# FocoosAI/focoos

Hardware: NVIDIA H100
Metric: images/sec fai-detr-l bs=32 640x640 inference (higher is better)
Workload: dtype f32 (storage and accumulation; every conv/linear product = 3 f16 wgmma products, error ~2^-21)

## Files before the change

### focoos_b200/csrc/conv_tc.cu

```cuda
#include <cuda.h>

#include <cstdlib>
#include <type_traits>

#include "common.cuh"
#include "tma.cuh"
#include "wgmma.cuh"

namespace fb200 {

namespace tc {

constexpr int BLOCK_M = 128;
constexpr int STAGING_BYTES = BLOCK_M * 128;
constexpr int NUM_THREADS = 384;
constexpr int CONSUMER_WARPS = 8;

struct PairOut { __half hi, lo; };
template <typename T> struct is_pair { static constexpr bool value = false; };
template <> struct is_pair<PairOut> { static constexpr bool value = true; };

struct KParams {
  const float* scale; const float* bias; const void* res;
  int act, Cout;
  int KH, KW, pad, cchunks;
  int w_batched;
  int lo_off;
  int w_seg;
  int BW, BH, tiles_w, tiles_h;
  int Ho, Wo;
  int x_pitch;
  int stride2;
  int num_k_blocks;
  int n_tiles, total_tiles;
  float* rowmax;
};

__device__ __forceinline__ void consumer_bar() { asm volatile("bar.sync 1, 256;" ::: "memory"); }

template <int BLOCK_K>
__device__ __forceinline__ uint64_t make_smem_desc(uint32_t smem_addr) {
  uint64_t d = 0;
  d |= (uint64_t)((smem_addr & 0x3FFFFu) >> 4);
  d |= (uint64_t)1 << 16;
  d |= (uint64_t)((8 * BLOCK_K * 2) >> 4) << 32;
  d |= (uint64_t)(BLOCK_K == 64 ? 1 : 2) << 62;
  return d;
}

template <bool GELU>
__device__ __forceinline__ float act1(float v, int act) {
  if constexpr (GELU) return 0.5f * v * (1.f + erff(v * 0.70710678118654752440f));
  switch (act & 15) {
    case FB200_ACT_RELU: return fmaxf(v, 0.f);
    case FB200_ACT_SILU: return __fdividef(v, 1.f + __expf(-v));
    default: return v;
  }
}

__device__ __forceinline__ void atomic_max_float(float* addr, float v) {
  if (v >= 0.f) atomicMax(reinterpret_cast<int*>(addr), __float_as_int(v));
  else atomicMin(reinterpret_cast<unsigned int*>(addr), __float_as_uint(v));
}

struct AccThread {
  int ct;
  int g;
  int r0;
  int cq;
};
__device__ __forceinline__ AccThread acc_thread() {
  const int ct = threadIdx.x - 128, lane = threadIdx.x & 31;
  return {ct, ct >> 7, (ct >> 7) * 64 + ((ct & 127) >> 5) * 16 + (lane >> 2), 2 * (lane & 3)};
}

template <typename TOut>
__device__ __forceinline__ int staging_offset(int row, int lc) {
  if constexpr (is_pair<TOut>::value) return row * 64 + ((((lc >> 3) ^ ((row >> 1) & 3)) << 4) | ((lc & 7) * 2));
  else if constexpr (sizeof(TOut) == 2) return row * 128 + ((((lc >> 3) ^ (row & 7)) << 4) | ((lc & 7) * 2));
  else return row * 128 + ((((lc >> 2) ^ (row & 7)) << 4) | ((lc & 3) * 4));
}

template <typename TOut>
__device__ __forceinline__ void staging_store(uint8_t* stg, int off, float v0, float v1) {
  if constexpr (is_pair<TOut>::value) {
    const __half2 hi = __floats2half2_rn(v0, v1);
    const float2 hf = __half22float2(hi);
    *reinterpret_cast<__half2*>(stg + off) = hi;
    *reinterpret_cast<__half2*>(stg + STAGING_BYTES / 2 + off) = __floats2half2_rn(v0 - hf.x, v1 - hf.y);
  } else if constexpr (sizeof(TOut) == 2) {
    *reinterpret_cast<__half2*>(stg + off) = __floats2half2_rn(v0, v1);
  } else {
    *reinterpret_cast<float2*>(stg + off) = make_float2(v0, v1);
  }
}

template <int NSTG, typename F>
__device__ __forceinline__ void staging_open(int ct, F&& then) {
  if (ct == 0) {
    tma_store_wait_read<NSTG - 1>();
    then();
  }
  consumer_bar();
}
template <typename TOut>
__device__ __forceinline__ void staging_close(int ct, const uint8_t* stg, const CUtensorMap* tmap_d, const CUtensorMap* tmap_d2, int n, int w0, int h0, int img) {
  fence_proxy_async();
  consumer_bar();
  if (ct == 0) {
    tma_store_4d(tmap_d, stg, n, w0, h0, img);
    if constexpr (is_pair<TOut>::value) tma_store_4d(tmap_d2, stg + STAGING_BYTES / 2, n, w0, h0, img);
    tma_store_commit();
  }
}

template <int BLOCK_K, bool FS> __host__ __device__ constexpr int a_stage_bytes() { return (FS ? 2 : 1) * BLOCK_M * BLOCK_K * 2; }
template <int BLOCK_N, int BLOCK_K, bool FS> __host__ __device__ constexpr int b_stage_bytes() { return (FS ? 2 : 1) * BLOCK_N * BLOCK_K * 2; }
template <int BLOCK_N, int STAGES, int BLOCK_K, int NSTG, bool FS> constexpr int smem_bytes() {
  return STAGES * (a_stage_bytes<BLOCK_K, FS>() + b_stage_bytes<BLOCK_N, BLOCK_K, FS>()) + NSTG * STAGING_BYTES + (2 * STAGES + 1) * 8 + 1024 ;
}

template <int BLOCK_N, int STAGES, typename TOut, int BLOCK_K, int NSTG, bool GELU, bool FS>
__global__ void __launch_bounds__(NUM_THREADS, 1)
conv_tc_kernel(const __grid_constant__ CUtensorMap tmap_a, const __grid_constant__ CUtensorMap tmap_b,
               const __grid_constant__ CUtensorMap tmap_d, const __grid_constant__ CUtensorMap tmap_r,
               const __grid_constant__ CUtensorMap tmap_d2, const __grid_constant__ CUtensorMap tmap_r2, const KParams p) {
  constexpr bool PAIR = is_pair<TOut>::value;
  static_assert(BLOCK_K == 32 || BLOCK_K == 64, "one swizzle row per channel chunk");
  extern __shared__ __align__(1024) uint8_t smem_raw[];
  uint8_t* smem = reinterpret_cast<uint8_t*>((reinterpret_cast<uintptr_t>(smem_raw) + 1023) & ~uintptr_t(1023));
  constexpr int A_STAGE_BYTES = a_stage_bytes<BLOCK_K, FS>();
  constexpr int B_STAGE_BYTES = b_stage_bytes<BLOCK_N, BLOCK_K, FS>();
  constexpr int A_HALF = BLOCK_M * BLOCK_K * 2;
  constexpr int B_HALF = BLOCK_N * BLOCK_K * 2;
  uint8_t* smem_a = smem;
  uint8_t* smem_b = smem + STAGES * A_STAGE_BYTES;
  uint8_t* staging = smem_b + STAGES * B_STAGE_BYTES;
  uint64_t* full_bar = reinterpret_cast<uint64_t*>(staging + NSTG * STAGING_BYTES);
  uint64_t* empty_bar = full_bar + STAGES;
  uint64_t* res_bar = empty_bar + STAGES;

  constexpr int CHUNK_COLS = 128 / (int)sizeof(TOut);
  constexpr int NCHUNKS = (BLOCK_N + CHUNK_COLS - 1) / CHUNK_COLS;
  constexpr int RES_SLOTS_A = A_STAGE_BYTES / STAGING_BYTES;
  constexpr int RES_SLOTS = RES_SLOTS_A + B_STAGE_BYTES / STAGING_BYTES;
  constexpr bool RES_RING = RES_SLOTS > 0;
  const bool res_ring = RES_RING && p.res != nullptr && p.rowmax == nullptr;
  auto res_slot = [&](int s, int slot) -> uint8_t* {
    return slot < RES_SLOTS_A ? smem_a + s * A_STAGE_BYTES + slot * STAGING_BYTES : smem_b + s * B_STAGE_BYTES + (slot - RES_SLOTS_A) * STAGING_BYTES;
  };
  auto chunks_of = [&](int n0) { return min(NCHUNKS, (p.Cout - n0 + CHUNK_COLS - 1) / CHUNK_COLS); };

  const int warp = threadIdx.x >> 5, lane = threadIdx.x & 31;
  if (threadIdx.x == 0) {
    asm volatile("prefetch.tensormap [%0];" ::"l"(&tmap_a) : "memory");
    asm volatile("prefetch.tensormap [%0];" ::"l"(&tmap_b) : "memory");
    asm volatile("prefetch.tensormap [%0];" ::"l"(&tmap_d) : "memory");
    for (int i = 0; i < STAGES; ++i) { mbar_init(&full_bar[i], 1); mbar_init(&empty_bar[i], CONSUMER_WARPS); }
    if constexpr (!RES_RING) mbar_init(res_bar, 1);
    fence_barrier_init();
  }
  __syncthreads();
  const int tiles_per_img = p.tiles_w * p.tiles_h;
  struct TileXY { int n0, img, h0, w0; };
  auto tile_of = [&](int t) {
    TileXY r;
    r.n0 = (t % p.n_tiles) * BLOCK_N;
    const int mt = t / p.n_tiles;
    r.img = mt / tiles_per_img;
    const int rem = mt - r.img * tiles_per_img;
    r.h0 = (rem / p.tiles_w) * p.BH;
    r.w0 = (rem % p.tiles_w) * p.BW;
    return r;
  };

  if (warp < 4) {
    if (threadIdx.x != 0) return;
    const uint32_t a_bytes = (uint32_t)(p.BW * p.BH * BLOCK_K * 2);
    auto load_a = [&](uint64_t* bar, void* dst, int c, int kh, int kw, int h0, int w0, int img) {
      if (!p.stride2) {
        tma_load_4d(&tmap_a, bar, dst, c, w0 + kw - p.pad, h0 + kh - p.pad, img);
      } else if (p.stride2 == 2) {
        tma_load_4d(&tmap_a, bar, dst, c, 2 * w0 + kw - p.pad, 2 * h0 + kh - p.pad, img);
      } else {
        const int th = kh - p.pad, tw = kw - p.pad;
        tma_load_5d(&tmap_a, bar, dst, (tw & 1) * p.x_pitch + c, w0 + (tw >> 1), th & 1, h0 + (th >> 1), img);
      }
    };
    auto load_b = [&](uint64_t* bar, void* dst, int k, int n0, int img) {
      if (p.w_batched) tma_load_3d(&tmap_b, bar, dst, k, n0, img);
      else tma_load_2d(&tmap_b, bar, dst, k, n0);
    };
    int stage = 0;
    uint32_t phase = 0;
    for (int t = blockIdx.x; t < p.total_tiles; t += gridDim.x) {
      const TileXY tc = tile_of(t);
      for (int kb = 0; kb < p.num_k_blocks; ++kb) {
        mbar_wait(&empty_bar[stage], phase ^ 1);
        const int tap = kb / p.cchunks, cc = kb - tap * p.cchunks;
        const int kh = tap / p.KW, kw = tap - kh * p.KW;
        uint8_t* dst_a = smem_a + stage * A_STAGE_BYTES;
        uint8_t* dst_b = smem_b + stage * B_STAGE_BYTES;
        if constexpr (FS) {
          const int k_hi = tap * 3 * p.w_seg + cc * BLOCK_K, k_lo = k_hi + p.w_seg;
          mbar_arrive_expect_tx(&full_bar[stage], 2u * a_bytes + (uint32_t)B_STAGE_BYTES);
          load_a(&full_bar[stage], dst_a, cc * BLOCK_K, kh, kw, tc.h0, tc.w0, tc.img);
          load_a(&full_bar[stage], dst_a + A_HALF, p.lo_off + cc * BLOCK_K, kh, kw, tc.h0, tc.w0, tc.img);
          load_b(&full_bar[stage], dst_b, k_hi, tc.n0, tc.img);
          load_b(&full_bar[stage], dst_b + B_HALF, k_lo, tc.n0, tc.img);
        } else {
          mbar_arrive_expect_tx(&full_bar[stage], a_bytes + (uint32_t)B_STAGE_BYTES);
          load_a(&full_bar[stage], dst_a, cc * BLOCK_K, kh, kw, tc.h0, tc.w0, tc.img);
          load_b(&full_bar[stage], dst_b, kb * BLOCK_K, tc.n0, tc.img);
        }
        if (++stage == STAGES) { stage = 0; phase ^= 1; }
      }
      if constexpr (RES_RING) if (res_ring) {
        const int nch = chunks_of(tc.n0);
        for (int ch = 0; ch < nch; ++ch) {
          const int slot = ch % RES_SLOTS;
          if (slot == 0) {
            mbar_wait(&empty_bar[stage], phase ^ 1);
            mbar_arrive_expect_tx(&full_bar[stage], (uint32_t)(min(RES_SLOTS, nch - ch) * p.BW * p.BH * 128));
          }
          uint8_t* dst = res_slot(stage, slot);
          tma_load_4d(&tmap_r, &full_bar[stage], dst, tc.n0 + ch * CHUNK_COLS, tc.w0, tc.h0, tc.img);
          if constexpr (PAIR) tma_load_4d(&tmap_r2, &full_bar[stage], dst + STAGING_BYTES / 2, tc.n0 + ch * CHUNK_COLS, tc.w0, tc.h0, tc.img);
          if (slot == RES_SLOTS - 1 || ch == nch - 1) {
            if (++stage == STAGES) { stage = 0; phase ^= 1; }
          }
        }
      }
    }
    return;
  }

  const AccThread th = acc_thread();
  constexpr int NACC = BLOCK_N / 2;
  const bool post = (p.act & FB200_ACT_RESIDUAL_AFTER) != 0;
  const bool has_res = p.res != nullptr;
  float acc[NACC];
  int stage = 0;
  uint32_t phase = 0, res_phase = 0, chunk_ctr = 0;
  for (int t = blockIdx.x; t < p.total_tiles; t += gridDim.x) {
    const TileXY tc = tile_of(t);
    int prev = -1;
    for (int kb = 0; kb < p.num_k_blocks; ++kb) {
      mbar_wait(&full_bar[stage], phase);
      const uint32_t sa = smem_u32(smem_a + stage * A_STAGE_BYTES) + (uint32_t)(th.g * 64 * BLOCK_K * 2);
      const uint32_t sb = smem_u32(smem_b + stage * B_STAGE_BYTES);
      const uint64_t da = make_smem_desc<BLOCK_K>(sa), db = make_smem_desc<BLOCK_K>(sb);
      wgmma_fence();
#pragma unroll
      for (int k = 0; k < BLOCK_K / 16; ++k) {
        const uint64_t ko = (uint64_t)(k * 2);
        Wgmma<BLOCK_N, 0>::mma(acc, da + ko, db + ko, (kb > 0 || k > 0) ? 1u : 0u);
        if constexpr (FS) {
          const uint64_t da_lo = make_smem_desc<BLOCK_K>(sa + A_HALF), db_lo = make_smem_desc<BLOCK_K>(sb + B_HALF);
          Wgmma<BLOCK_N, 0>::mma(acc, da + ko, db_lo + ko, 1u);
          Wgmma<BLOCK_N, 0>::mma(acc, da_lo + ko, db + ko, 1u);
        }
      }
      wgmma_commit();
      wgmma_wait<1>();
      if (prev >= 0 && lane == 0) mbar_arrive(&empty_bar[prev]);
      prev = stage;
      if (++stage == STAGES) { stage = 0; phase ^= 1; }
    }
    wgmma_wait<0>();
    if (prev >= 0 && lane == 0) mbar_arrive(&empty_bar[prev]);

    auto scale_of = [&](int n) { return (p.scale && n < p.Cout) ? __ldg(p.scale + n) : 1.f; };
    auto bias_of = [&](int n) { return (p.bias && n < p.Cout) ? __ldg(p.bias + n) : 0.f; };
    auto row_valid = [&](int row, int64_t& pix) {
      const int bh = row / p.BW, bw = row - bh * p.BW;
      const int ho = tc.h0 + bh, wo = tc.w0 + bw;
      pix = ((int64_t)tc.img * p.Ho + ho) * p.Wo + wo;
      return row < p.BW * p.BH && ho < p.Ho && wo < p.Wo;
    };
    if (p.rowmax) {
      float m[2] = {-INFINITY, -INFINITY};
#pragma unroll
      for (int j = 0; j < BLOCK_N / 8; ++j) {
#pragma unroll
        for (int e = 0; e < 2; ++e) {
          const int n = tc.n0 + 8 * j + th.cq + e;
          if (n < p.Cout) {
            const float s = scale_of(n), b = bias_of(n);
            m[0] = fmaxf(m[0], fmaf(acc[4 * j + e], s, b));
            m[1] = fmaxf(m[1], fmaf(acc[4 * j + 2 + e], s, b));
          }
        }
      }
#pragma unroll
      for (int h = 0; h < 2; ++h) {
        m[h] = fmaxf(m[h], __shfl_xor_sync(0xffffffffu, m[h], 1));
        m[h] = fmaxf(m[h], __shfl_xor_sync(0xffffffffu, m[h], 2));
        int64_t pix;
        if ((lane & 3) == 0 && row_valid(th.r0 + 8 * h, pix)) atomic_max_float(p.rowmax + pix, m[h]);
      }
      continue;
    }
    const int nch = chunks_of(tc.n0);
#pragma unroll
    for (int ch = 0; ch < NCHUNKS; ++ch) {
      const int c0 = ch * CHUNK_COLS;
      if (ch >= nch) break;
      uint8_t* stg = staging + (chunk_ctr % NSTG) * STAGING_BYTES;
      const uint8_t* res = stg;
      staging_open<NSTG>(th.ct, [&] {
        if constexpr (!RES_RING) if (has_res) {
          mbar_arrive_expect_tx(res_bar, (uint32_t)(p.BW * p.BH * 128));
          tma_load_4d(&tmap_r, res_bar, stg, tc.n0 + c0, tc.w0, tc.h0, tc.img);
          if constexpr (PAIR) tma_load_4d(&tmap_r2, res_bar, stg + STAGING_BYTES / 2, tc.n0 + c0, tc.w0, tc.h0, tc.img);
        }
      });
      if constexpr (RES_RING) {
        if (res_ring) {
          if (ch % RES_SLOTS == 0) mbar_wait(&full_bar[stage], phase);
          res = res_slot(stage, ch % RES_SLOTS);
        }
      } else if (has_res) {
        mbar_wait(res_bar, res_phase);
        res_phase ^= 1;
      }
#pragma unroll
      for (int jj = 0; jj < CHUNK_COLS / 8; ++jj) {
        const int j = c0 / 8 + jj;
        if (j >= BLOCK_N / 8) break;
        const int lc = 8 * jj + th.cq;
        const int n = tc.n0 + c0 + lc;
        const float s0 = scale_of(n), s1 = scale_of(n + 1), b0 = bias_of(n), b1 = bias_of(n + 1);
#pragma unroll
        for (int h = 0; h < 2; ++h) {
          const int row = th.r0 + 8 * h;
          float v0 = fmaf(acc[4 * j + 2 * h], s0, b0), v1 = fmaf(acc[4 * j + 2 * h + 1], s1, b1);
          const int off = staging_offset<TOut>(row, lc);
          auto add_residual = [&]() {
            if (!has_res) return;
            if constexpr (PAIR) {
              const float2 fh = __half22float2(*reinterpret_cast<const __half2*>(res + off));
              const float2 fl = __half22float2(*reinterpret_cast<const __half2*>(res + STAGING_BYTES / 2 + off));
              v0 += fh.x + fl.x;
              v1 += fh.y + fl.y;
            } else if constexpr (sizeof(TOut) == 2) {
              const float2 f = __half22float2(*reinterpret_cast<const __half2*>(res + off));
              v0 += f.x;
              v1 += f.y;
            } else {
              const float2 f = *reinterpret_cast<const float2*>(res + off);
              v0 += f.x;
              v1 += f.y;
            }
          };
          if (!post) add_residual();
          v0 = act1<GELU>(v0, p.act);
          v1 = act1<GELU>(v1, p.act);
          if (post) add_residual();
          staging_store<TOut>(stg, off, v0, v1);
        }
      }
      if constexpr (RES_RING) {
        if (res_ring && (ch % RES_SLOTS == RES_SLOTS - 1 || ch == nch - 1)) {
          __syncwarp();
          if (lane == 0) mbar_arrive(&empty_bar[stage]);
          if (++stage == STAGES) { stage = 0; phase ^= 1; }
        }
      }
      staging_close<TOut>(th.ct, stg, &tmap_d, &tmap_d2, tc.n0 + c0, tc.w0, tc.h0, tc.img);
      ++chunk_ctr;
    }
  }
  if (th.ct == 0) tma_store_wait_all();
}

constexpr int SC_BW = 16, SC_BH = 8;
constexpr int SC_BOX_ROWS = SC_BW * (SC_BH + 2);
constexpr int SC_BOX_BYTES = SC_BOX_ROWS * 64;
constexpr int SC_STAGE_BYTES = 2 * 3 * SC_BOX_BYTES;
constexpr int SC_STAGES = 2;
template <int BLOCK_N> __host__ __device__ constexpr int sc_w_bytes() { return 9 * 2 * BLOCK_N * 64; }
template <int BLOCK_N> constexpr int sc_smem_bytes() {
  return sc_w_bytes<BLOCK_N>() + SC_STAGES * SC_STAGE_BYTES + 2 * STAGING_BYTES + (2 * SC_STAGES + 1) * 8 + 1024 ;
}

template <int BLOCK_N, typename TOut>
__global__ void __launch_bounds__(NUM_THREADS, 1)
conv_tc_smallc_kernel(const __grid_constant__ CUtensorMap tmap_a, const __grid_constant__ CUtensorMap tmap_b,
                      const __grid_constant__ CUtensorMap tmap_d, const __grid_constant__ CUtensorMap tmap_d2, const KParams p) {
  constexpr int W_BYTES = sc_w_bytes<BLOCK_N>();
  constexpr int W_TAP = 2 * BLOCK_N * 64;
  extern __shared__ __align__(1024) uint8_t smem_raw[];
  uint8_t* smem = reinterpret_cast<uint8_t*>((reinterpret_cast<uintptr_t>(smem_raw) + 1023) & ~uintptr_t(1023));
  uint8_t* smem_w = smem;
  uint8_t* smem_a = smem_w + W_BYTES;
  uint8_t* staging = smem_a + SC_STAGES * SC_STAGE_BYTES;
  uint64_t* full_bar = reinterpret_cast<uint64_t*>(staging + 2 * STAGING_BYTES);
  uint64_t* empty_bar = full_bar + SC_STAGES;
  uint64_t* w_bar = empty_bar + SC_STAGES;
  constexpr int CHUNK_COLS = 32;
  constexpr int NCHUNKS = BLOCK_N / CHUNK_COLS;

  const int warp = threadIdx.x >> 5, lane = threadIdx.x & 31;
  if (threadIdx.x == 0) {
    asm volatile("prefetch.tensormap [%0];" ::"l"(&tmap_a) : "memory");
    asm volatile("prefetch.tensormap [%0];" ::"l"(&tmap_d) : "memory");
    for (int i = 0; i < SC_STAGES; ++i) { mbar_init(&full_bar[i], 1); mbar_init(&empty_bar[i], CONSUMER_WARPS); }
    mbar_init(w_bar, 1);
    fence_barrier_init();
  }
  __syncthreads();
  const int tiles_per_img = p.tiles_w * p.tiles_h;
  struct TileXY { int img, h0, w0; };
  auto tile_of = [&](int t) {
    TileXY r;
    r.img = t / tiles_per_img;
    const int rem = t - r.img * tiles_per_img;
    r.h0 = (rem / p.tiles_w) * SC_BH;
    r.w0 = (rem % p.tiles_w) * SC_BW;
    return r;
  };

  if (warp < 4) {
    if (threadIdx.x != 0) return;
    mbar_arrive_expect_tx(w_bar, (uint32_t)W_BYTES);
    for (int tap = 0; tap < 9; ++tap) {
      tma_load_2d(&tmap_b, w_bar, smem_w + tap * W_TAP, tap * 3 * p.w_seg, 0);
      tma_load_2d(&tmap_b, w_bar, smem_w + tap * W_TAP + W_TAP / 2, tap * 3 * p.w_seg + p.w_seg, 0);
    }
    int stage = 0;
    uint32_t phase = 0;
    for (int t = blockIdx.x; t < p.total_tiles; t += gridDim.x) {
      const TileXY tc = tile_of(t);
      mbar_wait(&empty_bar[stage], phase ^ 1);
      mbar_arrive_expect_tx(&full_bar[stage], (uint32_t)SC_STAGE_BYTES);
      uint8_t* dst = smem_a + stage * SC_STAGE_BYTES;
      for (int kw = 0; kw < 3; ++kw) {
        tma_load_4d(&tmap_a, &full_bar[stage], dst + kw * SC_BOX_BYTES, 0, tc.w0 + kw - 1, tc.h0 - 1, tc.img);
        tma_load_4d(&tmap_a, &full_bar[stage], dst + (3 + kw) * SC_BOX_BYTES, p.lo_off, tc.w0 + kw - 1, tc.h0 - 1, tc.img);
      }
      if (++stage == SC_STAGES) { stage = 0; phase ^= 1; }
    }
    return;
  }

  const AccThread th = acc_thread();
  float acc[BLOCK_N / 2];
  float sc[BLOCK_N / 4], bi[BLOCK_N / 4];
#pragma unroll
  for (int j = 0; j < BLOCK_N / 8; ++j)
#pragma unroll
    for (int e = 0; e < 2; ++e) {
      const int n = 8 * j + th.cq + e;
      sc[2 * j + e] = p.scale ? __ldg(p.scale + n) : 1.f;
      bi[2 * j + e] = p.bias ? __ldg(p.bias + n) : 0.f;
    }
  mbar_wait(w_bar, 0);
  const uint32_t sw = smem_u32(smem_w);
  int stage = 0;
  uint32_t phase = 0, chunk_ctr = 0;
  for (int t = blockIdx.x; t < p.total_tiles; t += gridDim.x) {
    const TileXY tc = tile_of(t);
    mbar_wait(&full_bar[stage], phase);
    const uint32_t sa = smem_u32(smem_a + stage * SC_STAGE_BYTES) + (uint32_t)(th.g * 64 * 64);
    wgmma_fence();
#pragma unroll
    for (int tap = 0; tap < 9; ++tap) {
      const int kh = tap / 3, kw = tap - 3 * (tap / 3);
      const uint32_t a_tap = sa + (uint32_t)(kw * SC_BOX_BYTES + kh * SC_BW * 64);
      const uint64_t da = make_smem_desc<32>(a_tap), da_lo = make_smem_desc<32>(a_tap + 3 * SC_BOX_BYTES);
      const uint64_t db = make_smem_desc<32>(sw + tap * W_TAP), db_lo = make_smem_desc<32>(sw + tap * W_TAP + W_TAP / 2);
#pragma unroll
      for (int k = 0; k < 2; ++k) {
        const uint64_t ko = (uint64_t)(k * 2);
        Wgmma<BLOCK_N, 0>::mma(acc, da + ko, db + ko, (tap > 0 || k > 0) ? 1u : 0u);
        Wgmma<BLOCK_N, 0>::mma(acc, da + ko, db_lo + ko, 1u);
        Wgmma<BLOCK_N, 0>::mma(acc, da_lo + ko, db + ko, 1u);
      }
    }
    wgmma_commit();
    wgmma_wait<0>();
    if (lane == 0) mbar_arrive(&empty_bar[stage]);
    if (++stage == SC_STAGES) { stage = 0; phase ^= 1; }

#pragma unroll
    for (int ch = 0; ch < NCHUNKS; ++ch) {
      uint8_t* stg = staging + (chunk_ctr & 1) * STAGING_BYTES;
      staging_open<2>(th.ct, [] {});
#pragma unroll
      for (int jj = 0; jj < CHUNK_COLS / 8; ++jj) {
        const int j = ch * (CHUNK_COLS / 8) + jj;
        const int lc = 8 * jj + th.cq;
#pragma unroll
        for (int h = 0; h < 2; ++h) {
          const int row = th.r0 + 8 * h;
          const float v0 = act1<false>(fmaf(acc[4 * j + 2 * h], sc[2 * j], bi[2 * j]), p.act);
          const float v1 = act1<false>(fmaf(acc[4 * j + 2 * h + 1], sc[2 * j + 1], bi[2 * j + 1]), p.act);
          staging_store<TOut>(stg, staging_offset<TOut>(row, lc), v0, v1);
        }
      }
      staging_close<TOut>(th.ct, stg, &tmap_d, &tmap_d2, ch * CHUNK_COLS, tc.w0, tc.h0, tc.img);
      ++chunk_ctr;
    }
  }
  if (th.ct == 0) tma_store_wait_all();
}

static void choose_tile(int Ho, int Wo, int* BW, int* BH) {
  double best = -1.0;
  for (int bw = 1; bw <= (Wo < 128 ? Wo : 128); ++bw) {
    int bh = 128 / bw;
    if (bh > Ho) bh = Ho;
    if (bh < 1) continue;
    const double tiles = (double)((Wo + bw - 1) / bw) * (double)((Ho + bh - 1) / bh);
    const double eff = (double)Wo * Ho / (tiles * 128.0);
    if (eff > best + 1e-9 || (eff > best - 1e-9 && bw > *BW)) { best = eff; *BW = bw; *BH = bh; }
  }
}

struct OutMaps { CUtensorMap d, d2, r, r2; };
static int encode_out_maps(OutMaps* m, const ConvParams& p, int Wo, int Ho, int B, int BW, int BH, uint64_t batch_stride) {
  const bool pair = p.out_dtype == FB200_F16PAIR, f32 = p.out_dtype == FB200_F32;
  const CUtensorMapDataType dt = f32 ? CU_TENSOR_MAP_DATA_TYPE_FLOAT32 : CU_TENSOR_MAP_DATA_TYPE_FLOAT16;
  const int elt = f32 ? 4 : 2;
  const CUtensorMapSwizzle swz = pair ? CU_TENSOR_MAP_SWIZZLE_64B : CU_TENSOR_MAP_SWIZZLE_128B;
  const uint64_t OP = (uint64_t)p.out_pitch, RP = (uint64_t)p.res_pitch;
  const uint64_t dims[4] = {(uint64_t)p.Cout, (uint64_t)Wo, (uint64_t)Ho, (uint64_t)B};
  const uint64_t str[4] = {1, OP, OP * Wo, batch_stride}, rstr[4] = {1, RP, RP * Wo, RP * Wo * Ho};
  const uint32_t box[4] = {(uint32_t)(pair || f32 ? 32 : 64), (uint32_t)BW, (uint32_t)BH, 1};
  int rc = encode(&m->d, dt, elt, 4, p.out, dims, str, box, pair ? "conv_tc: D(hi)" : "conv_tc: D", swz);
  if (rc) return rc;
  m->d2 = m->d;
  if (pair) rc = encode(&m->d2, dt, elt, 4, static_cast<__half*>(p.out) + p.out_lo_off, dims, str, box, "conv_tc: D(lo)", swz);
  if (rc) return rc;
  m->r = m->d; m->r2 = m->d2;
  if (!p.res) return FB200_OK;
  rc = encode(&m->r, dt, elt, 4, const_cast<void*>(p.res), dims, rstr, box, pair ? "conv_tc: R(hi)" : "conv_tc: R", swz);
  if (rc || !pair) return rc;
  return encode(&m->r2, dt, elt, 4, const_cast<__half*>(static_cast<const __half*>(p.res)) + p.res_lo_off, dims, rstr, box, "conv_tc: R(lo)", swz);
}

static bool smallc_fits(const ConvParams& p) {
  return p.split3 && p.Cin == 3 * 32 && (p.Cout == 32 || p.Cout == 64) && p.KH == 3 && p.KW == 3 && p.stride == 1 && p.pad == 1 &&
         !p.res && !p.rowmax && p.w_bs == 0 && (p.out_dtype == FB200_F32 || p.out_dtype == FB200_F16PAIR);
}

static int conv2d_tc_smallc(const ConvParams& p, cudaStream_t st) {
  KParams kp{};
  kp.scale = p.scale; kp.bias = p.bias; kp.act = p.act; kp.Cout = p.Cout;
  kp.lo_off = (int)p.x_lo_off;
  kp.w_seg = 32;
  kp.tiles_w = (p.Wo + SC_BW - 1) / SC_BW; kp.tiles_h = (p.Ho + SC_BH - 1) / SC_BH; kp.Ho = p.Ho; kp.Wo = p.Wo;
  const int64_t total = (int64_t)p.B * kp.tiles_w * kp.tiles_h;
  if (total > 0x7fffffffLL) { set_error("conv_tc: too many tiles (%lld)", (long long)total); return FB200_ERR_UNSUPPORTED; }
  kp.total_tiles = (int)total;
  CUtensorMap ta, tb;
  OutMaps om;
  const uint64_t P = (uint64_t)p.x_pitch;
  {
    const uint64_t dims[4] = {(uint64_t)kp.lo_off + 32, (uint64_t)p.W, (uint64_t)p.H, (uint64_t)p.B};
    const uint64_t str[4] = {1, P, P * p.W, P * p.W * p.H};
    const uint32_t box[4] = {32, SC_BW, SC_BH + 2, 1};
    int rc = encode(&ta, CU_TENSOR_MAP_DATA_TYPE_FLOAT16, 2, 4, const_cast<void*>(p.x), dims, str, box, "conv_tc: A(patch)", CU_TENSOR_MAP_SWIZZLE_64B);
    if (rc) return rc;
  }
  {
    const uint64_t dims[2] = {(uint64_t)p.K, (uint64_t)p.Cout};
    const uint64_t str[2] = {1, (uint64_t)p.K};
    const uint32_t box[2] = {32, (uint32_t)p.Cout};
    int rc = encode(&tb, CU_TENSOR_MAP_DATA_TYPE_FLOAT16, 2, 2, const_cast<void*>(p.w), dims, str, box, "conv_tc: W", CU_TENSOR_MAP_SWIZZLE_64B);
    if (rc) return rc;
  }
  if (int rc = encode_out_maps(&om, p, p.Wo, p.Ho, p.B, SC_BW, SC_BH, (uint64_t)p.out_bs)) return rc;
  auto run = [&](auto blockn_tag, auto out_tag) -> int {
    constexpr int BN_ = decltype(blockn_tag)::value;
    return launch_persistent<conv_tc_smallc_kernel<BN_, decltype(out_tag)>, sc_smem_bytes<BN_>()>("conv_tc_smallc_kernel", kp.total_tiles, NUM_THREADS, st, ta, tb,
                                                                                                 om.d, om.d2, kp);
  };
  typedef std::integral_constant<int, 32> N32;
  typedef std::integral_constant<int, 64> N64;
  const bool outp = p.out_dtype == FB200_F16PAIR;
  if (p.Cout == 32) return outp ? run(N32{}, PairOut{}) : run(N32{}, float{});
  return outp ? run(N64{}, PairOut{}) : run(N64{}, float{});
}

}

bool conv2d_tc_supported(const ConvParams& p, int x_dtype, int out_dtype) {
  if (x_dtype != FB200_F16) return false;
  if (out_dtype != FB200_F16 && out_dtype != FB200_F32 && out_dtype != FB200_F16PAIR) return false;
  if (p.split3 && out_dtype == FB200_F16) return false;
  const int Clog = p.split3 ? p.Cin / 3 : p.Cin;
  if (out_dtype == FB200_F16PAIR) {
    if (!p.split3 || p.rowmax || p.w_bs != 0 || p.Cout % 8 != 0) return false;
    if ((p.out_lo_off * 2) % 16 != 0 || (p.out_pitch * 2) % 16 != 0 || (p.out_bs * 2) % 16 != 0) return false;
    if (p.res && ((p.res_lo_off * 2) % 16 != 0 || (p.res_pitch * 2) % 16 != 0 || p.Cout % 32 != 0)) return false;
  }
  if (p.split3 && (p.x_lo_off * 2) % 16 != 0) return false;
  if (Clog % 32 != 0 || p.x_pitch % 8 != 0) return false;
  if (p.split3 && p.Cin % 3 != 0) return false;
  if ((reinterpret_cast<uintptr_t>(p.x) | reinterpret_cast<uintptr_t>(p.w) | reinterpret_cast<uintptr_t>(p.out)) & 15) return false;
  const int oelt = out_dtype == FB200_F32 ? 4 : 2;
  if ((p.out_pitch * oelt) % 16 != 0) return false;
  if (!p.rowmax && (p.Cout * oelt) % 16 != 0) return false;
  if (p.res && ((p.res_pitch * oelt) % 16 != 0 || (reinterpret_cast<uintptr_t>(p.res) & 15))) return false;
  if (p.res && out_dtype != FB200_F16PAIR && p.Cout % (128 / oelt) != 0) return false;
  if (p.KH != p.KW) return false;
  if (p.w_bs != 0 && (p.w_bs * 2) % 16 != 0) return false;
  if ((p.act & 15) == FB200_ACT_GELU && (out_dtype != FB200_F16 || Clog % 64 != 0)) return false;
  if ((p.act & 15) == FB200_ACT_SIGMOID) return false;
  if ((p.out_bs * oelt) % 16 != 0) return false;
  if (p.stride == 1) return (2 * p.pad == p.KH - 1) || (p.KH == 1 && p.pad == 0);
  if (p.stride == 2) {
    if (p.KH == 3 && p.pad == 1) return true;
    return p.KH == 2 && p.pad == 0 && p.H % 2 == 0 && p.W % 2 == 0;
  }
  return false;
}

int conv2d_tc(const ConvParams& p, cudaStream_t st) {
  using namespace tc;
  if (smallc_fits(p)) return conv2d_tc_smallc(p, st);
  KParams kp;
  kp.scale = p.scale; kp.bias = p.bias; kp.res = p.res; kp.act = p.act; kp.Cout = p.Cout;
  kp.KH = p.KH; kp.KW = p.KW; kp.pad = p.pad;
  const int Clog = p.split3 ? p.Cin / 3 : p.Cin;
  const int BK = (Clog % 64 == 0) ? 64 : 32;
  kp.lo_off = p.split3 ? (int)p.x_lo_off : Clog;
  kp.w_seg = Clog;
  const CUtensorMapSwizzle swz = BK == 64 ? CU_TENSOR_MAP_SWIZZLE_128B : CU_TENSOR_MAP_SWIZZLE_64B;
  kp.cchunks = Clog / BK; kp.x_pitch = p.x_pitch;
  kp.stride2 = (p.stride != 2) ? 0 : (p.H % 2 == 0 && p.W % 2 == 0) ? 1 : 2;
  kp.num_k_blocks = p.KH * p.KW * kp.cchunks;
  int B = p.B, H = p.H, W = p.W, Ho = p.Ho, Wo = p.Wo;
  const bool flat = (p.KH == 1 && p.stride == 1 && p.out_bs == (int64_t)p.Ho * p.Wo * p.out_pitch) && p.w_bs == 0;
  kp.w_batched = p.w_bs != 0 ? 1 : 0;
  kp.rowmax = p.rowmax;
  if (flat) {
    if (p.M > 0x7fffffffLL) { set_error("conv_tc: M too large"); return FB200_ERR_UNSUPPORTED; }
    W = Wo = (int)p.M; H = Ho = 1; B = 1;
  }
  int BW = 1, BH = 1;
  choose_tile(Ho, Wo, &BW, &BH);
  kp.BW = BW; kp.BH = BH; kp.tiles_w = (Wo + BW - 1) / BW; kp.tiles_h = (Ho + BH - 1) / BH; kp.Ho = Ho; kp.Wo = Wo;
  const int64_t m_tiles = (int64_t)B * kp.tiles_w * kp.tiles_h;

  CUtensorMap ta, tb;
  OutMaps om;
  int rc;
  const uint64_t P = (uint64_t)p.x_pitch;
  if (!kp.stride2) {
    const uint64_t dims[4] = {(uint64_t)(p.split3 ? kp.lo_off + Clog : p.Cin), (uint64_t)W, (uint64_t)H, (uint64_t)B};
    const uint64_t str[4] = {1, P, P * W, P * W * H};
    const uint32_t box[4] = {(uint32_t)BK, (uint32_t)BW, (uint32_t)BH, 1};
    rc = encode(&ta, CU_TENSOR_MAP_DATA_TYPE_FLOAT16, 2, 4, const_cast<void*>(p.x), dims, str, box, "conv_tc: A", swz);
  } else if (kp.stride2 == 2) {
    const uint64_t dims[4] = {(uint64_t)(p.split3 ? kp.lo_off + Clog : p.Cin), (uint64_t)W, (uint64_t)H, (uint64_t)B};
    const uint64_t str[4] = {1, P, P * W, P * W * H};
    const uint32_t box[4] = {(uint32_t)BK, 2 * (uint32_t)BW, 2 * (uint32_t)BH, 1};
    const uint32_t estr[4] = {1, 2, 2, 1};
    rc = encode(&ta, CU_TENSOR_MAP_DATA_TYPE_FLOAT16, 2, 4, const_cast<void*>(p.x), dims, str, box, "conv_tc: A(s2 odd)", swz, estr);
  } else {
    const uint64_t dims[5] = {2 * P, (uint64_t)W / 2, 2, (uint64_t)H / 2, (uint64_t)B};
    const uint64_t str[5] = {1, 2 * P, P * W, 2 * P * W, P * W * H};
    const uint32_t box[5] = {(uint32_t)BK, (uint32_t)BW, 1, (uint32_t)BH, 1};
    rc = encode(&ta, CU_TENSOR_MAP_DATA_TYPE_FLOAT16, 2, 5, const_cast<void*>(p.x), dims, str, box, "conv_tc: A(s2)", swz);
  }
  if (rc) return rc;
  rc = encode_out_maps(&om, p, Wo, Ho, B, BW, BH, flat ? (uint64_t)p.out_pitch * Wo * Ho : (uint64_t)p.out_bs);
  if (rc) return rc;

  auto run = [&](auto blockn_tag, auto stages_tag, auto bk_tag, auto gelu_tag, auto fs_tag) -> int {
    constexpr bool FS_ = decltype(fs_tag)::value;
    constexpr int BN_ = decltype(blockn_tag)::value;
    constexpr int ST_ = decltype(stages_tag)::value;
    constexpr int BK_ = decltype(bk_tag)::value;
    constexpr int NS_ = 2;
    {
      const uint64_t dims[3] = {(uint64_t)p.K, (uint64_t)p.Cout, (uint64_t)p.B};
      const uint64_t str[3] = {1, (uint64_t)p.K, (uint64_t)p.w_bs};
      const uint32_t box[3] = {(uint32_t)BK_, (uint32_t)BN_, 1};
      int r2 = encode(&tb, CU_TENSOR_MAP_DATA_TYPE_FLOAT16, 2, p.w_bs ? 3 : 2, const_cast<void*>(p.w), dims, str, box, "conv_tc: W", swz);
      if (r2) return r2;
    }
    kp.n_tiles = (p.Cout + BN_ - 1) / BN_;
    const int64_t total = m_tiles * kp.n_tiles;
    if (total > 0x7fffffffLL) { set_error("conv_tc: too many tiles (%lld)", (long long)total); return FB200_ERR_UNSUPPORTED; }
    kp.total_tiles = (int)total;
    auto launch = [&](auto out_tag) -> int {
      return launch_persistent<conv_tc_kernel<BN_, ST_, decltype(out_tag), BK_, NS_, decltype(gelu_tag)::value, FS_>, smem_bytes<BN_, ST_, BK_, NS_, FS_>()>(
          "conv_tc_kernel", kp.total_tiles, NUM_THREADS, st, ta, tb, om.d, om.r, om.d2, om.r2, kp);
    };
    const bool outp = p.out_dtype == FB200_F16PAIR;
    if constexpr (decltype(gelu_tag)::value) return launch(__half{});
    else if constexpr (FS_) return outp ? launch(PairOut{}) : launch(float{});
    else {
      if (outp) { set_error("conv_tc: pair output is only produced by the fused-split configurations"); return FB200_ERR_UNSUPPORTED; }
      return p.out_dtype == FB200_F16 ? launch(__half{}) : launch(float{});
    }
  };
  using std::integral_constant;
  typedef std::false_type NF;
  typedef std::true_type FS;
  typedef integral_constant<int, 64> K64;
  typedef integral_constant<int, 32> K32;
  typedef integral_constant<int, 128> N128;
  typedef integral_constant<int, 64> N64;
  typedef integral_constant<int, 4> S4;
  typedef integral_constant<int, 3> S3;
  if ((p.act & 15) == FB200_ACT_GELU)
    return run(N128{}, S4{}, K64{}, std::true_type{}, NF{});
  if (p.split3) {
    if (BK == 64) {
      if (p.Cout > 64) return run(N128{}, S3{}, K64{}, std::false_type{}, FS{});
      return run(N64{}, S4{}, K64{}, std::false_type{}, FS{});
    }
    if (p.Cout > 64) return run(N128{}, S4{}, K32{}, std::false_type{}, FS{});
    return run(N64{}, S4{}, K32{}, std::false_type{}, FS{});
  }
  if (BK == 32) {
    if (p.Cout > 64) return run(N128{}, S4{}, K32{}, std::false_type{}, NF{});
    return run(N64{}, S4{}, K32{}, std::false_type{}, NF{});
  }
  if (p.Cout > 64) return run(N128{}, S4{}, K64{}, std::false_type{}, NF{});
  return run(N64{}, S4{}, K64{}, std::false_type{}, NF{});
}

}
```

Before: 905.1.

## Ping-pong consumer warpgroups with register reallocation in conv TC kernel

Measured after the change: 982.8, median of 6. 8.6% higher.

```diff
diff --git a/focoos_b200/csrc/conv_tc.cu b/focoos_b200/csrc/conv_tc.cu
--- a/focoos_b200/csrc/conv_tc.cu
+++ b/focoos_b200/csrc/conv_tc.cu
@@ -15,6 +15,8 @@
 constexpr int STAGING_BYTES = BLOCK_M * 128;
 constexpr int NUM_THREADS = 384;
 constexpr int CONSUMER_WARPS = 8;
+constexpr int GROUP_WARPS = 4;
+constexpr int PRODUCER_REGS = 40, CONSUMER_REGS = 232;
 
 struct PairOut { __half hi, lo; };
 template <typename T> struct is_pair { static constexpr bool value = false; };
@@ -36,7 +38,29 @@
   float* rowmax;
 };
 
-__device__ __forceinline__ void consumer_bar() { asm volatile("bar.sync 1, 256;" ::: "memory"); }
+__device__ __forceinline__ void bar_sync(int id, int n) { asm volatile("bar.sync %0, %1;" ::"r"(id), "r"(n) : "memory"); }
+__device__ __forceinline__ void bar_arrive(int id, int n) { asm volatile("bar.arrive %0, %1;" ::"r"(id), "r"(n) : "memory"); }
+template <int REGS> __device__ __forceinline__ void regs_dec() { asm volatile("setmaxnreg.dec.sync.aligned.u32 %0;" ::"n"(REGS)); }
+template <int REGS> __device__ __forceinline__ void regs_inc() { asm volatile("setmaxnreg.inc.sync.aligned.u32 %0;" ::"n"(REGS)); }
+
+__device__ __forceinline__ uint32_t sreg_tid() {
+  uint32_t v;
+  asm volatile("mov.u32 %0, %%tid.x;" : "=r"(v));
+  return v;
+}
+__device__ __forceinline__ int grid_ctas() {
+  uint32_t v;
+  asm volatile("mov.u32 %0, %%nctaid.x;" : "=r"(v));
+  return (int)v;
+}
+__device__ __forceinline__ int pp_row() { const uint32_t t = sreg_tid(); return (int)((t & 127) >> 5) * 16 + (int)((t & 31) >> 2); }
+__device__ __forceinline__ int pp_col() { return 2 * (int)(sreg_tid() & 3); }
+
+struct Team {
+  bool issuer;
+  int bar, n;
+  __device__ __forceinline__ void sync() const { bar_sync(bar, n); }
+};
 
 template <int BLOCK_K>
 __device__ __forceinline__ uint64_t make_smem_desc(uint32_t smem_addr) {
@@ -81,33 +105,36 @@
   else return row * 128 + ((((lc >> 2) ^ (row & 7)) << 4) | ((lc & 3) * 4));
 }
 
+__device__ __forceinline__ uint32_t h2_bits(__half2 h) { return *reinterpret_cast<uint32_t*>(&h); }
+__device__ __forceinline__ void sts_b32(uint32_t a, uint32_t v) { asm volatile("st.shared.b32 [%0], %1;" ::"r"(a), "r"(v) : "memory"); }
+__device__ __forceinline__ void sts_f2(uint32_t a, float x, float y) { asm volatile("st.shared.v2.f32 [%0], {%1, %2};" ::"r"(a), "f"(x), "f"(y) : "memory"); }
 template <typename TOut>
-__device__ __forceinline__ void staging_store(uint8_t* stg, int off, float v0, float v1) {
+__device__ __forceinline__ void staging_store(uint32_t stg, int off, float v0, float v1) {
   if constexpr (is_pair<TOut>::value) {
     const __half2 hi = __floats2half2_rn(v0, v1);
     const float2 hf = __half22float2(hi);
-    *reinterpret_cast<__half2*>(stg + off) = hi;
-    *reinterpret_cast<__half2*>(stg + STAGING_BYTES / 2 + off) = __floats2half2_rn(v0 - hf.x, v1 - hf.y);
+    sts_b32(stg + off, h2_bits(hi));
+    sts_b32(stg + STAGING_BYTES / 2 + off, h2_bits(__floats2half2_rn(v0 - hf.x, v1 - hf.y)));
   } else if constexpr (sizeof(TOut) == 2) {
-    *reinterpret_cast<__half2*>(stg + off) = __floats2half2_rn(v0, v1);
+    sts_b32(stg + off, h2_bits(__floats2half2_rn(v0, v1)));
   } else {
-    *reinterpret_cast<float2*>(stg + off) = make_float2(v0, v1);
+    sts_f2(stg + off, v0, v1);
   }
 }
 
 template <int NSTG, typename F>
-__device__ __forceinline__ void staging_open(int ct, F&& then) {
-  if (ct == 0) {
+__device__ __forceinline__ void staging_open(const Team& tm, F&& then) {
+  if (tm.issuer) {
     tma_store_wait_read<NSTG - 1>();
     then();
   }
-  consumer_bar();
+  tm.sync();
 }
 template <typename TOut>
-__device__ __forceinline__ void staging_close(int ct, const uint8_t* stg, const CUtensorMap* tmap_d, const CUtensorMap* tmap_d2, int n, int w0, int h0, int img) {
+__device__ __forceinline__ void staging_close(const Team& tm, const uint8_t* stg, const CUtensorMap* tmap_d, const CUtensorMap* tmap_d2, int n, int w0, int h0, int img) {
   fence_proxy_async();
-  consumer_bar();
-  if (ct == 0) {
+  tm.sync();
+  if (tm.issuer) {
     tma_store_4d(tmap_d, stg, n, w0, h0, img);
     if constexpr (is_pair<TOut>::value) tma_store_4d(tmap_d2, stg + STAGING_BYTES / 2, n, w0, h0, img);
     tma_store_commit();
@@ -127,6 +154,7 @@
                const __grid_constant__ CUtensorMap tmap_d2, const __grid_constant__ CUtensorMap tmap_r2, const KParams p) {
   constexpr bool PAIR = is_pair<TOut>::value;
   static_assert(BLOCK_K == 32 || BLOCK_K == 64, "one swizzle row per channel chunk");
+  static_assert(NSTG == 2, "one staging buffer per consumer warp-group");
   extern __shared__ __align__(1024) uint8_t smem_raw[];
   uint8_t* smem = reinterpret_cast<uint8_t*>((reinterpret_cast<uintptr_t>(smem_raw) + 1023) & ~uintptr_t(1023));
   constexpr int A_STAGE_BYTES = a_stage_bytes<BLOCK_K, FS>();
@@ -138,17 +166,9 @@
   uint8_t* staging = smem_b + STAGES * B_STAGE_BYTES;
   uint64_t* full_bar = reinterpret_cast<uint64_t*>(staging + NSTG * STAGING_BYTES);
   uint64_t* empty_bar = full_bar + STAGES;
-  uint64_t* res_bar = empty_bar + STAGES;
-
   constexpr int CHUNK_COLS = 128 / (int)sizeof(TOut);
   constexpr int NCHUNKS = (BLOCK_N + CHUNK_COLS - 1) / CHUNK_COLS;
-  constexpr int RES_SLOTS_A = A_STAGE_BYTES / STAGING_BYTES;
-  constexpr int RES_SLOTS = RES_SLOTS_A + B_STAGE_BYTES / STAGING_BYTES;
-  constexpr bool RES_RING = RES_SLOTS > 0;
-  const bool res_ring = RES_RING && p.res != nullptr && p.rowmax == nullptr;
-  auto res_slot = [&](int s, int slot) -> uint8_t* {
-    return slot < RES_SLOTS_A ? smem_a + s * A_STAGE_BYTES + slot * STAGING_BYTES : smem_b + s * B_STAGE_BYTES + (slot - RES_SLOTS_A) * STAGING_BYTES;
-  };
+  constexpr int ROW_BYTES = PAIR ? 64 : 128;
   auto chunks_of = [&](int n0) { return min(NCHUNKS, (p.Cout - n0 + CHUNK_COLS - 1) / CHUNK_COLS); };
 
   const int warp = threadIdx.x >> 5, lane = threadIdx.x & 31;
@@ -156,8 +176,7 @@
     asm volatile("prefetch.tensormap [%0];" ::"l"(&tmap_a) : "memory");
     asm volatile("prefetch.tensormap [%0];" ::"l"(&tmap_b) : "memory");
     asm volatile("prefetch.tensormap [%0];" ::"l"(&tmap_d) : "memory");
-    for (int i = 0; i < STAGES; ++i) { mbar_init(&full_bar[i], 1); mbar_init(&empty_bar[i], CONSUMER_WARPS); }
-    if constexpr (!RES_RING) mbar_init(res_bar, 1);
+    for (int i = 0; i < STAGES; ++i) { mbar_init(&full_bar[i], 1); mbar_init(&empty_bar[i], GROUP_WARPS); }
     fence_barrier_init();
   }
   __syncthreads();
@@ -175,6 +194,7 @@
   };
 
   if (warp < 4) {
+    regs_dec<PRODUCER_REGS>();
     if (threadIdx.x != 0) return;
     const uint32_t a_bytes = (uint32_t)(p.BW * p.BH * BLOCK_K * 2);
     auto load_a = [&](uint64_t* bar, void* dst, int c, int kh, int kw, int h0, int w0, int img) {
@@ -215,6 +235,250 @@
         }
         if (++stage == STAGES) { stage = 0; phase ^= 1; }
       }
+    }
+    return;
+  }
+
+  regs_inc<CONSUMER_REGS>();
+  const int g = (threadIdx.x - 128) >> 7;
+  const Team team{(threadIdx.x & 127) == 0, 2 + g, 128};
+  uint8_t* stg = staging + g * STAGING_BYTES;
+  constexpr int NACC = BLOCK_N / 2;
+  float acc[2][NACC];
+  int stage = 0;
+  uint32_t phase = 0;
+  for (int t = blockIdx.x + g * grid_ctas(); t < p.total_tiles; t += 2 * grid_ctas()) {
+    if (t != blockIdx.x) {
+      stage += p.num_k_blocks;
+      phase ^= (uint32_t)((stage / STAGES) & 1);
+      stage %= STAGES;
+      bar_sync(4 + g, 256);
+    }
+    for (int kb = 0; kb < p.num_k_blocks; ++kb) {
+      mbar_wait(&full_bar[stage], phase);
+      const uint32_t sa = smem_u32(smem_a + stage * A_STAGE_BYTES);
+      const uint32_t sb = smem_u32(smem_b + stage * B_STAGE_BYTES);
+      const uint64_t da = make_smem_desc<BLOCK_K>(sa), db = make_smem_desc<BLOCK_K>(sb);
+      wgmma_fence();
+#pragma unroll
+      for (int k = 0; k < BLOCK_K / 16; ++k) {
+        const uint64_t ko = (uint64_t)(k * 2);
+#pragma unroll
+        for (int hf = 0; hf < 2; ++hf) {
+          const uint64_t dah = da + (uint64_t)(hf * 64 * BLOCK_K * 2 / 16) + ko;
+          Wgmma<BLOCK_N, 0>::mma(acc[hf], dah, db + ko, (kb > 0 || k > 0) ? 1u : 0u);
+          if constexpr (FS) {
+            Wgmma<BLOCK_N, 0>::mma(acc[hf], dah, db + (uint64_t)(B_HALF / 16) + ko, 1u);
+            Wgmma<BLOCK_N, 0>::mma(acc[hf], dah + (uint64_t)(A_HALF / 16), db + ko, 1u);
+          }
+        }
+      }
+      wgmma_commit();
+      wgmma_wait<1>();
+      if (kb > 0 && lane == 0) mbar_arrive(&empty_bar[stage == 0 ? STAGES - 1 : stage - 1]);
+      if (++stage == STAGES) { stage = 0; phase ^= 1; }
+    }
+    if (t + grid_ctas() < p.total_tiles) bar_arrive(4 + (g ^ 1), 256);
+    wgmma_wait<0>();
+    if (lane == 0) mbar_arrive(&empty_bar[stage == 0 ? STAGES - 1 : stage - 1]);
+
+    const TileXY tc = tile_of(t);
+    auto scale_of = [&](int n) { return (p.scale && n < p.Cout) ? __ldg(p.scale + n) : 1.f; };
+    auto bias_of = [&](int n) { return (p.bias && n < p.Cout) ? __ldg(p.bias + n) : 0.f; };
+    auto row_valid = [&](int row, int64_t& pix) {
+      const int bh = row / p.BW, bw = row - bh * p.BW;
+      const int ho = tc.h0 + bh, wo = tc.w0 + bw;
+      pix = ((int64_t)tc.img * p.Ho + ho) * p.Wo + wo;
+      return row < p.BW * p.BH && ho < p.Ho && wo < p.Wo;
+    };
+    if (p.rowmax) {
+      const int r0 = pp_row(), cq = pp_col();
+      float m[2][2] = {{-INFINITY, -INFINITY}, {-INFINITY, -INFINITY}};
+#pragma unroll
+      for (int j = 0; j < BLOCK_N / 8; ++j) {
+#pragma unroll
+        for (int e = 0; e < 2; ++e) {
+          const int n = tc.n0 + 8 * j + cq + e;
+          if (n < p.Cout) {
+            const float s = scale_of(n), b = bias_of(n);
+#pragma unroll
+            for (int hf = 0; hf < 2; ++hf) {
+              m[hf][0] = fmaxf(m[hf][0], fmaf(acc[hf][4 * j + e], s, b));
+              m[hf][1] = fmaxf(m[hf][1], fmaf(acc[hf][4 * j + 2 + e], s, b));
+            }
+          }
+        }
+      }
+#pragma unroll
+      for (int hf = 0; hf < 2; ++hf)
+#pragma unroll
+        for (int h = 0; h < 2; ++h) {
+          m[hf][h] = fmaxf(m[hf][h], __shfl_xor_sync(0xffffffffu, m[hf][h], 1));
+          m[hf][h] = fmaxf(m[hf][h], __shfl_xor_sync(0xffffffffu, m[hf][h], 2));
+          int64_t pix;
+          if ((lane & 3) == 0 && row_valid(64 * hf + r0 + 8 * h, pix)) atomic_max_float(p.rowmax + pix, m[hf][h]);
+        }
+      continue;
+    }
+    const int nch = chunks_of(tc.n0);
+#pragma unroll
+    for (int ch = 0; ch < NCHUNKS; ++ch) {
+      const int c0 = ch * CHUNK_COLS;
+      if (ch >= nch) break;
+      staging_open<1>(team, [] {});
+      const uint32_t out = smem_u32(stg);
+#pragma unroll
+      for (int jj = 0; jj < CHUNK_COLS / 8; ++jj) {
+        const int j = c0 / 8 + jj;
+        if (j >= BLOCK_N / 8) break;
+        const int r0 = pp_row(), cq = pp_col();
+        const int lc = 8 * jj + cq;
+        const int n = tc.n0 + c0 + lc;
+        const float s0 = scale_of(n), s1 = scale_of(n + 1), b0 = bias_of(n), b1 = bias_of(n + 1);
+        const int off0 = staging_offset<TOut>(r0, lc);
+#pragma unroll
+        for (int hf = 0; hf < 2; ++hf)
+#pragma unroll
+          for (int h = 0; h < 2; ++h) {
+            const float v0 = act1<GELU>(fmaf(acc[hf][4 * j + 2 * h], s0, b0), p.act);
+            const float v1 = act1<GELU>(fmaf(acc[hf][4 * j + 2 * h + 1], s1, b1), p.act);
+            staging_store<TOut>(out, off0 + (64 * hf + 8 * h) * ROW_BYTES, v0, v1);
+          }
+      }
+      staging_close<TOut>(team, stg, &tmap_d, &tmap_d2, tc.n0 + c0, tc.w0, tc.h0, tc.img);
+    }
+  }
+  if (team.issuer) tma_store_wait_all();
+}
+
+__device__ __forceinline__ void consumer_bar() { asm volatile("bar.sync 1, 256;" ::: "memory"); }
+template <typename TOut>
+__device__ __forceinline__ void coop_staging_store(uint8_t* stg, int off, float v0, float v1) {
+  if constexpr (is_pair<TOut>::value) {
+    const __half2 hi = __floats2half2_rn(v0, v1);
+    const float2 hf = __half22float2(hi);
+    *reinterpret_cast<__half2*>(stg + off) = hi;
+    *reinterpret_cast<__half2*>(stg + STAGING_BYTES / 2 + off) = __floats2half2_rn(v0 - hf.x, v1 - hf.y);
+  } else if constexpr (sizeof(TOut) == 2) {
+    *reinterpret_cast<__half2*>(stg + off) = __floats2half2_rn(v0, v1);
+  } else {
+    *reinterpret_cast<float2*>(stg + off) = make_float2(v0, v1);
+  }
+}
+template <int NSTG, typename F>
+__device__ __forceinline__ void coop_staging_open(int ct, F&& then) {
+  if (ct == 0) {
+    tma_store_wait_read<NSTG - 1>();
+    then();
+  }
+  consumer_bar();
+}
+template <typename TOut>
+__device__ __forceinline__ void coop_staging_close(int ct, const uint8_t* stg, const CUtensorMap* tmap_d, const CUtensorMap* tmap_d2, int n, int w0, int h0, int img) {
+  fence_proxy_async();
+  consumer_bar();
+  if (ct == 0) {
+    tma_store_4d(tmap_d, stg, n, w0, h0, img);
+    if constexpr (is_pair<TOut>::value) tma_store_4d(tmap_d2, stg + STAGING_BYTES / 2, n, w0, h0, img);
+    tma_store_commit();
+  }
+}
+
+template <int BLOCK_N, int STAGES, typename TOut, int BLOCK_K, int NSTG, bool GELU, bool FS>
+__global__ void __launch_bounds__(NUM_THREADS, 1)
+conv_tc_kernel_coop(const __grid_constant__ CUtensorMap tmap_a, const __grid_constant__ CUtensorMap tmap_b,
+               const __grid_constant__ CUtensorMap tmap_d, const __grid_constant__ CUtensorMap tmap_r,
+               const __grid_constant__ CUtensorMap tmap_d2, const __grid_constant__ CUtensorMap tmap_r2, const KParams p) {
+  constexpr bool PAIR = is_pair<TOut>::value;
+  static_assert(BLOCK_K == 32 || BLOCK_K == 64, "one swizzle row per channel chunk");
+  extern __shared__ __align__(1024) uint8_t smem_raw[];
+  uint8_t* smem = reinterpret_cast<uint8_t*>((reinterpret_cast<uintptr_t>(smem_raw) + 1023) & ~uintptr_t(1023));
+  constexpr int A_STAGE_BYTES = a_stage_bytes<BLOCK_K, FS>();
+  constexpr int B_STAGE_BYTES = b_stage_bytes<BLOCK_N, BLOCK_K, FS>();
+  constexpr int A_HALF = BLOCK_M * BLOCK_K * 2;
+  constexpr int B_HALF = BLOCK_N * BLOCK_K * 2;
+  uint8_t* smem_a = smem;
+  uint8_t* smem_b = smem + STAGES * A_STAGE_BYTES;
+  uint8_t* staging = smem_b + STAGES * B_STAGE_BYTES;
+  uint64_t* full_bar = reinterpret_cast<uint64_t*>(staging + NSTG * STAGING_BYTES);
+  uint64_t* empty_bar = full_bar + STAGES;
+  uint64_t* res_bar = empty_bar + STAGES;
+
+  constexpr int CHUNK_COLS = 128 / (int)sizeof(TOut);
+  constexpr int NCHUNKS = (BLOCK_N + CHUNK_COLS - 1) / CHUNK_COLS;
+  constexpr int RES_SLOTS_A = A_STAGE_BYTES / STAGING_BYTES;
+  constexpr int RES_SLOTS = RES_SLOTS_A + B_STAGE_BYTES / STAGING_BYTES;
+  constexpr bool RES_RING = RES_SLOTS > 0;
+  const bool res_ring = RES_RING && p.res != nullptr && p.rowmax == nullptr;
+  auto res_slot = [&](int s, int slot) -> uint8_t* {
+    return slot < RES_SLOTS_A ? smem_a + s * A_STAGE_BYTES + slot * STAGING_BYTES : smem_b + s * B_STAGE_BYTES + (slot - RES_SLOTS_A) * STAGING_BYTES;
+  };
+  auto chunks_of = [&](int n0) { return min(NCHUNKS, (p.Cout - n0 + CHUNK_COLS - 1) / CHUNK_COLS); };
+
+  const int warp = threadIdx.x >> 5, lane = threadIdx.x & 31;
+  if (threadIdx.x == 0) {
+    asm volatile("prefetch.tensormap [%0];" ::"l"(&tmap_a) : "memory");
+    asm volatile("prefetch.tensormap [%0];" ::"l"(&tmap_b) : "memory");
+    asm volatile("prefetch.tensormap [%0];" ::"l"(&tmap_d) : "memory");
+    for (int i = 0; i < STAGES; ++i) { mbar_init(&full_bar[i], 1); mbar_init(&empty_bar[i], CONSUMER_WARPS); }
+    if constexpr (!RES_RING) mbar_init(res_bar, 1);
+    fence_barrier_init();
+  }
+  __syncthreads();
+  const int tiles_per_img = p.tiles_w * p.tiles_h;
+  struct TileXY { int n0, img, h0, w0; };
+  auto tile_of = [&](int t) {
+    TileXY r;
+    r.n0 = (t % p.n_tiles) * BLOCK_N;
+    const int mt = t / p.n_tiles;
+    r.img = mt / tiles_per_img;
+    const int rem = mt - r.img * tiles_per_img;
+    r.h0 = (rem / p.tiles_w) * p.BH;
+    r.w0 = (rem % p.tiles_w) * p.BW;
+    return r;
+  };
+
+  if (warp < 4) {
+    if (threadIdx.x != 0) return;
+    const uint32_t a_bytes = (uint32_t)(p.BW * p.BH * BLOCK_K * 2);
+    auto load_a = [&](uint64_t* bar, void* dst, int c, int kh, int kw, int h0, int w0, int img) {
+      if (!p.stride2) {
+        tma_load_4d(&tmap_a, bar, dst, c, w0 + kw - p.pad, h0 + kh - p.pad, img);
+      } else if (p.stride2 == 2) {
+        tma_load_4d(&tmap_a, bar, dst, c, 2 * w0 + kw - p.pad, 2 * h0 + kh - p.pad, img);
+      } else {
+        const int th = kh - p.pad, tw = kw - p.pad;
+        tma_load_5d(&tmap_a, bar, dst, (tw & 1) * p.x_pitch + c, w0 + (tw >> 1), th & 1, h0 + (th >> 1), img);
+      }
+    };
+    auto load_b = [&](uint64_t* bar, void* dst, int k, int n0, int img) {
+      if (p.w_batched) tma_load_3d(&tmap_b, bar, dst, k, n0, img);
+      else tma_load_2d(&tmap_b, bar, dst, k, n0);
+    };
+    int stage = 0;
+    uint32_t phase = 0;
+    for (int t = blockIdx.x; t < p.total_tiles; t += gridDim.x) {
+      const TileXY tc = tile_of(t);
+      for (int kb = 0; kb < p.num_k_blocks; ++kb) {
+        mbar_wait(&empty_bar[stage], phase ^ 1);
+        const int tap = kb / p.cchunks, cc = kb - tap * p.cchunks;
+        const int kh = tap / p.KW, kw = tap - kh * p.KW;
+        uint8_t* dst_a = smem_a + stage * A_STAGE_BYTES;
+        uint8_t* dst_b = smem_b + stage * B_STAGE_BYTES;
+        if constexpr (FS) {
+          const int k_hi = tap * 3 * p.w_seg + cc * BLOCK_K, k_lo = k_hi + p.w_seg;
+          mbar_arrive_expect_tx(&full_bar[stage], 2u * a_bytes + (uint32_t)B_STAGE_BYTES);
+          load_a(&full_bar[stage], dst_a, cc * BLOCK_K, kh, kw, tc.h0, tc.w0, tc.img);
+          load_a(&full_bar[stage], dst_a + A_HALF, p.lo_off + cc * BLOCK_K, kh, kw, tc.h0, tc.w0, tc.img);
+          load_b(&full_bar[stage], dst_b, k_hi, tc.n0, tc.img);
+          load_b(&full_bar[stage], dst_b + B_HALF, k_lo, tc.n0, tc.img);
+        } else {
+          mbar_arrive_expect_tx(&full_bar[stage], a_bytes + (uint32_t)B_STAGE_BYTES);
+          load_a(&full_bar[stage], dst_a, cc * BLOCK_K, kh, kw, tc.h0, tc.w0, tc.img);
+          load_b(&full_bar[stage], dst_b, kb * BLOCK_K, tc.n0, tc.img);
+        }
+        if (++stage == STAGES) { stage = 0; phase ^= 1; }
+      }
       if constexpr (RES_RING) if (res_ring) {
         const int nch = chunks_of(tc.n0);
         for (int ch = 0; ch < nch; ++ch) {
@@ -308,7 +572,7 @@
       if (ch >= nch) break;
       uint8_t* stg = staging + (chunk_ctr % NSTG) * STAGING_BYTES;
       const uint8_t* res = stg;
-      staging_open<NSTG>(th.ct, [&] {
+      coop_staging_open<NSTG>(th.ct, [&] {
         if constexpr (!RES_RING) if (has_res) {
           mbar_arrive_expect_tx(res_bar, (uint32_t)(p.BW * p.BH * 128));
           tma_load_4d(&tmap_r, res_bar, stg, tc.n0 + c0, tc.w0, tc.h0, tc.img);
@@ -357,7 +621,7 @@
           v0 = act1<GELU>(v0, p.act);
           v1 = act1<GELU>(v1, p.act);
           if (post) add_residual();
-          staging_store<TOut>(stg, off, v0, v1);
+          coop_staging_store<TOut>(stg, off, v0, v1);
         }
       }
       if constexpr (RES_RING) {
@@ -367,7 +631,7 @@
           if (++stage == STAGES) { stage = 0; phase ^= 1; }
         }
       }
-      staging_close<TOut>(th.ct, stg, &tmap_d, &tmap_d2, tc.n0 + c0, tc.w0, tc.h0, tc.img);
+      coop_staging_close<TOut>(th.ct, stg, &tmap_d, &tmap_d2, tc.n0 + c0, tc.w0, tc.h0, tc.img);
       ++chunk_ctr;
     }
   }
@@ -445,6 +709,7 @@
   }
 
   const AccThread th = acc_thread();
+  const Team team{th.ct == 0, 1, 256};
   float acc[BLOCK_N / 2];
   float sc[BLOCK_N / 4], bi[BLOCK_N / 4];
 #pragma unroll
@@ -486,7 +751,7 @@
 #pragma unroll
     for (int ch = 0; ch < NCHUNKS; ++ch) {
       uint8_t* stg = staging + (chunk_ctr & 1) * STAGING_BYTES;
-      staging_open<2>(th.ct, [] {});
+      staging_open<2>(team, [] {});
 #pragma unroll
       for (int jj = 0; jj < CHUNK_COLS / 8; ++jj) {
         const int j = ch * (CHUNK_COLS / 8) + jj;
@@ -496,10 +761,10 @@
           const int row = th.r0 + 8 * h;
           const float v0 = act1<false>(fmaf(acc[4 * j + 2 * h], sc[2 * j], bi[2 * j]), p.act);
           const float v1 = act1<false>(fmaf(acc[4 * j + 2 * h + 1], sc[2 * j + 1], bi[2 * j + 1]), p.act);
-          staging_store<TOut>(stg, staging_offset<TOut>(row, lc), v0, v1);
-        }
-      }
-      staging_close<TOut>(th.ct, stg, &tmap_d, &tmap_d2, ch * CHUNK_COLS, tc.w0, tc.h0, tc.img);
+          staging_store<TOut>(smem_u32(stg), staging_offset<TOut>(row, lc), v0, v1);
+        }
+      }
+      staging_close<TOut>(team, stg, &tmap_d, &tmap_d2, ch * CHUNK_COLS, tc.w0, tc.h0, tc.img);
       ++chunk_ctr;
     }
   }
@@ -688,7 +953,12 @@
     if (total > 0x7fffffffLL) { set_error("conv_tc: too many tiles (%lld)", (long long)total); return FB200_ERR_UNSUPPORTED; }
     kp.total_tiles = (int)total;
     auto launch = [&](auto out_tag) -> int {
-      return launch_persistent<conv_tc_kernel<BN_, ST_, decltype(out_tag), BK_, NS_, decltype(gelu_tag)::value, FS_>, smem_bytes<BN_, ST_, BK_, NS_, FS_>()>(
+      constexpr bool GE_ = decltype(gelu_tag)::value;
+      typedef decltype(out_tag) TO_;
+      if (p.res && !p.rowmax)
+        return launch_persistent<conv_tc_kernel_coop<BN_, ST_, TO_, BK_, NS_, GE_, FS_>, smem_bytes<BN_, ST_, BK_, NS_, FS_>()>(
+            "conv_tc_kernel_coop", kp.total_tiles, NUM_THREADS, st, ta, tb, om.d, om.r, om.d2, om.r2, kp);
+      return launch_persistent<conv_tc_kernel<BN_, ST_, TO_, BK_, NS_, GE_, FS_>, smem_bytes<BN_, ST_, BK_, NS_, FS_>()>(
           "conv_tc_kernel", kp.total_tiles, NUM_THREADS, st, ta, tb, om.d, om.r, om.d2, om.r2, kp);
     };
     const bool outp = p.out_dtype == FB200_F16PAIR;
```
